# ucl-exoplanets/wayne

Measured on AMD Instinct MI355X. Metric: simulated WFC3-IR exposures/sec (1014x1014, NSAMP=16, spatial scan), higher is better.
Workload: dtype k_ramp<float, true, 1, false, true>: exact integer sums (int64 accumulators + int32 sky counts) then an all-f32 per-read chain; f32 thrower (int32 LDS tiles -> int64 fixed-point accumulators, 2^-28 e-); f32 reads; 1 GPU; cfg4: G141 spatial scan 5 px/s, SUBARRAY=1024 (frame 1014x1014), SPARS10 NSAMP=16, K=128 sub-samples, W=4494 bins, 9.92e+08 electrons/exposure, all detector effects on (flat, sky, cosmic rays, gain, dark, non-linearity, clip, read noise), thrower=split (wide component per electron, narrow component multinomial), f32 reads (the default of ExposureGenerator, Observation, VisitRunner and the CLI), on; exposures_per_rank=2241

## Files before the change

### wayne_amd/_lib.py

```python
import ctypes as C
import os
import threading
import weakref

import numpy as np

from . import build as _build

OK, E_INVALID, E_NEGATIVE, E_OVERFLOW, E_NOMEM, E_HIP, E_NODEVICE, E_STATE = 0, -1, -2, -3, -4, -5, -6, -7
RNG_REPLAY, RNG_PHILOX, RNG_SPLIT = 0, 1, 2
F_ADD_FLAT = 1 << 0
F_ADD_GAIN_VARIATIONS = 1 << 1
F_ADD_NON_LINEAR = 1 << 2
F_CLIP_DET_LIMITS = 1 << 3
F_ADD_READ_NOISE = 1 << 4
F_ADD_STELLAR_NOISE = 1 << 5
F_ADD_DARK = 1 << 6
F_ADD_INITIAL_BIAS = 1 << 7
F_OUT_F64 = 1 << 16
F_OUT_U16 = 1 << 18
OUT_FLAGS = {np.dtype(np.float32): 0, np.dtype(np.float64): F_OUT_F64, np.dtype(np.uint16): F_OUT_U16}
F_EXACT_SAMPLERS = 1 << 17
PROF_KERNELS = 8
ABI_VERSION = 7
# ... 33 lines not shown


class ExposureDesc(C.Structure):
    _fields_ = [("seed", C.c_uint32), ("exposure_index", C.c_uint32), ("rng_mode", C.c_int),
                ("threads_compat", C.c_int), ("flags", C.c_uint32), ("sub_scale", C.c_int),
                ("n_wl", C.c_int), ("wl_um", _dp), ("flux", _dp), ("depth", _dp),
                ("n_samples", C.c_int), ("x_ref", _dp), ("y_ref", _dp), ("dur_ms", _dp),
                ("replay_seed", _ip), ("sample_read", _ip),
                ("n_reads", C.c_int), ("read_dt_s", _dp),
                ("sky_ct_s", C.c_double), ("cosmic_rate", C.c_double), ("scale_factor", C.c_double),
                ("noise_mean", C.c_double), ("noise_std", C.c_double),
                ("thrower_margin", C.c_int), ("thrower_splits", C.c_int),
                ("lc_z", _dp), ("lc_hidden", _dp), ("lc_rp", _dp), ("lc_ld", C.c_double * 4)]


class SourceDesc(C.Structure):
    _fields_ = [("tag", C.c_uint32), ("n_wl", C.c_int), ("wl_um", _dp), ("flux", _dp),
                ("dx", C.c_double), ("dy", C.c_double)]


class TrapDesc(C.Structure):
    _fields_ = [("n_traps", C.c_double * 2), ("efficiency", C.c_double * 2), ("lifetime_s", C.c_double * 2),
                ("n_rate", C.c_int), ("rate_lo", C.c_double), ("rate_hi", C.c_double), ("start", _dp * 2)]


class ExtractDesc(C.Structure):
    _fields_ = [("steps", C.c_uint32), ("row_lo", C.c_int * EXTRACT_PRODUCTS), ("row_hi", C.c_int * EXTRACT_PRODUCTS),
                ("bg_col_lo", C.c_int), ("bg_col_hi", C.c_int)]


class Profile(C.Structure):
    _fields_ = [("name", C.c_char_p * PROF_KERNELS), ("launches", C.c_uint64 * PROF_KERNELS),
                ("ms", C.c_double * PROF_KERNELS), ("electrons", C.c_uint64)]


_vp = C.c_void_p
SYMBOLS = {
    "wayne_abi_version": (C.c_int, []),
    "wayne_strerror": (C.c_char_p, [C.c_int]),
    "wayne_build_flags": (C.c_char_p, []),
    "wayne_device_count": (C.c_int, []),
    "wayne_ctx_create": (_vp, [C.c_int, C.POINTER(C.c_int)]),
    "wayne_ctx_destroy": (None, [_vp]),
    "wayne_last_error": (C.c_char_p, [_vp]),
    "wayne_ctx_synchronize": (C.c_int, [_vp]),
    "wayne_ctx_stream": (_vp, [_vp]),
    "wayne_ctx_set_knob": (C.c_int, [_vp, C.c_char_p, C.c_longlong]),
    "wayne_ctx_get_knob": (C.c_int, [_vp, C.c_char_p, C.POINTER(C.c_longlong)]),
    "wayne_psf_apply": (C.c_int, [_vp, _vp, C.c_int, _vp, _vp, _vp, _vp, _vp, C.c_int, C.c_int,
                                  C.c_uint32, C.c_int, C.c_int, C.c_uint32, C.c_uint32, _vp]),
    "wayne_psf_apply_ex": (C.c_int, [_vp, _vp, C.c_int, _vp, _vp, _vp, _vp, _vp, C.c_int, C.c_int,
                                     C.c_uint32, C.c_int, C.c_int, C.c_uint32, C.c_uint32, C.c_uint32, _vp]),
    "wayne_ctx_set_grism": (C.c_int, [_vp, C.POINTER(GrismDesc)]),
    "wayne_ctx_set_calibration": (C.c_int, [_vp, C.POINTER(Calibration)]),
    "wayne_ctx_slots": (C.c_int, [_vp]),
    "wayne_exposure_upload": (C.c_int, [_vp, C.c_int, C.POINTER(ExposureDesc)]),
    "wayne_exposure_run": (C.c_int, [_vp, C.c_int]),
    "wayne_exposure_run_checked": (C.c_int, [_vp, C.c_int]),
    "wayne_exposure_status": (C.c_int, [_vp, C.c_int, C.POINTER(C.c_int)]),
    "wayne_ctx_reruns": (C.c_ulonglong, [_vp]),
    "wayne_exposure_download": (C.c_int, [_vp, C.c_int, _vp]),
    "wayne_exposure_fetch_async": (C.c_int, [_vp, C.c_int]),
    "wayne_exposure_wait": (C.c_int, [_vp, C.c_int, C.POINTER(C.c_void_p)]),
    "wayne_exposure_device_reads": (_vp, [_vp, C.c_int]),
    "wayne_exposure_synthesize": (C.c_int, [_vp, C.POINTER(ExposureDesc), _vp]),
    "wayne_exposure_debug_fetch": (C.c_int, [_vp, C.c_int, _vp, _vp, _vp, _vp]),
    "wayne_exposure_debug_depth": (C.c_int, [_vp, C.c_int, _vp]),
    "wayne_exposure_debug_boxes": (C.c_int, [_vp, C.c_int, _vp, _vp, C.POINTER(C.c_int)]),
    "wayne_exposure_run_front": (C.c_int, [_vp, C.c_int]),
    "wayne_exposure_run_back": (C.c_int, [_vp, C.c_int]),
    "wayne_exposure_ramp_variant": (C.c_int, [_vp, C.c_int, C.c_char_p, C.c_int]),
    "wayne_exposure_set_sources": (C.c_int, [_vp, C.c_int, C.POINTER(SourceDesc), C.c_int]),
    "wayne_source_seed": (C.c_uint32, [C.c_uint32, C.c_uint32]),
    "wayne_exposure_set_traps": (C.c_int, [_vp, C.c_int, C.POINTER(TrapDesc)]),
    "wayne_exposure_debug_fetch_source": (C.c_int, [_vp, C.c_int, C.c_int, _vp, _vp, _vp]),
    "wayne_exposure_set_extraction": (C.c_int, [_vp, C.c_int, C.POINTER(ExtractDesc)]),
    "wayne_exposure_fetch_spectra_async": (C.c_int, [_vp, C.c_int]),
    "wayne_exposure_wait_spectra": (C.c_int, [_vp, C.c_int, C.POINTER(_dp), C.POINTER(_dp)]),
    "wayne_exposure_download_spectra": (C.c_int, [_vp, C.c_int, _vp, _vp]),
    "wayne_extract_profile": (C.c_int, [_vp, C.POINTER(C.c_uint64), C.POINTER(C.c_double)]),
    "wayne_profile_enable": (C.c_int, [_vp, C.c_int]),
    "wayne_profile_select": (C.c_int, [_vp, C.c_uint]),
    "wayne_profile_reset": (C.c_int, [_vp]),
    "wayne_profile_get": (C.c_int, [_vp, C.POINTER(Profile)]),
    "wayne_philox4x32": (None, [_vp, _vp, _vp]),
    "wayne_host_sample_draws": (None, [C.c_uint32, C.c_uint32, C.c_int, _vp, _vp, _vp]),
}

_lib = None


def load():
    global _lib, _lib_path
    if _lib is None:
        path = _build.LIB
        override = os.environ.get("WAYNE_HIP_LIB")
        if override:
            path = override
        elif _build.stale():
            if os.path.exists(_build.HIPCC):
                _build.build(verbose=False)
            elif not os.path.exists(path):
                raise ImportError("libwayne_hip.so is not built and hipcc is unavailable (%s)" % _build.HIPCC)
        L = C.CDLL(path)
        for name, (res, args) in SYMBOLS.items():
            f = getattr(L, name)
            f.restype = res
            f.argtypes = args
        if L.wayne_abi_version() != ABI_VERSION:
            raise ImportError("libwayne_hip.so ABI version mismatch")
        flags = L.wayne_build_flags().decode().split()
        if flags and os.environ.get("WAYNE_ALLOW_FLAGGED_LIB", "") != "1":
            raise ImportError("%s was built with %s: not the product's library (tests and measurement scripts that mean "
                              "to load it set WAYNE_ALLOW_FLAGGED_LIB=1)" % (path, " ".join(flags)))
        _lib = L
        _lib_path = path
    return _lib


_lib_path = None


def library_info():
    L = load()
    return _lib_path or _build.LIB, L.wayne_build_flags().decode().strip()


def ptr(a, ctype=None):
    if a is None:
        return None
    assert a.flags["C_CONTIGUOUS"]
    if ctype is None:
        return a.ctypes.data_as(C.c_void_p)
    return a.ctypes.data_as(C.POINTER(ctype))


def out_dtype_of(flags):
    return np.dtype(np.float64 if flags & F_OUT_F64 else np.uint16 if flags & F_OUT_U16 else np.float32)


def f64(a):
    return np.ascontiguousarray(a, dtype=np.float64)


def f32(a):
    return np.ascontiguousarray(a, dtype=np.float32)


def i32(a):
    return np.ascontiguousarray(a, dtype=np.int32)


KNOBS = ("tile_ints", "batch", "thin", "no_acc_box", "lane_reach", "throw_wgs", "keep_narrow", "no_fuse", "fork_narrow",
         "streams", "upload_timing", "ramp_reads")
_live_contexts = weakref.WeakSet()
_knob_defaults = {}


def set_knob_all(name, value):
    if name not in KNOBS:
        raise KeyError("no knob named %r" % (name,))
    if value is None:
        _knob_defaults.pop(name, None)
    else:
        _knob_defaults[name] = int(value)
    for c in list(_live_contexts):
        if getattr(c, "_h", None):
            c.set_knob(name, value)


def reset_knobs_all():
    for name in list(_knob_defaults):
        set_knob_all(name, None)


class Context(object):

    def __init__(self, device=0):
        self._L = load()
        st = C.c_int(0)
        self._h = self._L.wayne_ctx_create(int(device), C.byref(st))
        if not self._h:
            msg = self._L.wayne_strerror(st.value).decode()
            cls = WayneNoDeviceError if st.value == E_NODEVICE else WayneError
            raise cls(st.value, "wayne_ctx_create(device=%d): %s -- the HIP path is the only path, "
                                "there is no CPU fallback" % (device, msg))
        self.device = device
        self._slot_meta = {}
        self._slot_src = {}
        _live_contexts.add(self)
        for name, value in _knob_defaults.items():
            self.set_knob(name, value)

    def close(self):
        if getattr(self, "_h", None):
            self._L.wayne_ctx_destroy(self._h)
            self._h = None

    def __del__(self):
        try:
            self.close()
        except Exception:
            pass

    def __enter__(self):
        return self

    def __exit__(self, *a):
        self.close()

    def check(self, status):
        if status != OK:
            raise WayneError(status, self._L.wayne_last_error(self._h).decode())

    def synchronize(self):
        self.check(self._L.wayne_ctx_synchronize(self._h))

    def set_knob(self, name, value):
        self.check(self._L.wayne_ctx_set_knob(self._h, name.encode(), -1 if value is None else int(value)))

    def get_knob(self, name):
        v = C.c_longlong(0)
        self.check(self._L.wayne_ctx_get_knob(self._h, name.encode(), C.byref(v)))
        return None if v.value < 0 else int(v.value)

    @property
    def stream(self):
        return self._L.wayne_ctx_stream(self._h)

    def psf_apply(self, counts, x, y, ratio, sl, sh, nr, nc, seed, threads=1, rng_mode=RNG_REPLAY,
                  exposure=0, subsample=0, exact_samplers=False):
        counts = i32(counts)
        x, y, ratio, sl, sh = f64(x), f64(y), f64(ratio), f64(sl), f64(sh)
        n = counts.size
        if not all(a.size == n for a in (x, y, ratio, sl, sh)):
            raise ValueError("apply_psf: arrays differ in length")
        out = np.empty(max(int(nr) * int(nc), 0), dtype=np.int32)
        self.check(self._L.wayne_psf_apply_ex(self._h, ptr(counts), n, ptr(x), ptr(y), ptr(ratio), ptr(sl),
                                              ptr(sh), int(nr), int(nc), int(seed) & 0xFFFFFFFF, int(threads),
                                              int(rng_mode), int(exposure), int(subsample),
                                              F_EXACT_SAMPLERS if exact_samplers else 0, ptr(out)))
        return out

    def set_grism(self, trace_coeff, wl_solution, psf_ratio_poly, psf_sigmal_poly, psf_sigmah_poly,
                  sens_wl_um, sens_val, flat_wmin, flat_wmax):
        g = GrismDesc()
        g.trace_coeff[:] = list(map(float, trace_coeff))
        g.wl_solution[:] = list(map(float, wl_solution))
        g.psf_ratio_poly[:] = list(map(float, psf_ratio_poly))
        g.psf_sigmal_poly[:] = list(map(float, psf_sigmal_poly))
        g.psf_sigmah_poly[:] = list(map(float, psf_sigmah_poly))
        wl, val = f64(sens_wl_um), f64(sens_val)
        if wl.size != val.size:
            raise ValueError("sensitivity table: wl and val differ in length")
        g.n_sens = wl.size
        g.sens_wl_um = ptr(wl, C.c_double)
        g.sens_val = ptr(val, C.c_double)
        g.flat_wmin, g.flat_wmax = float(flat_wmin), float(flat_wmax)
        self.check(self._L.wayne_ctx_set_grism(self._h, C.byref(g)))

    def set_calibration(self, subarray, n_reads, flat=None, pfl=None, sky=None, lin=None, dark_sci=None,
                        dark_err=None, zero_read=None):
        N = 1014 if subarray == 1024 else subarray
        S = N + 10
        k = Calibration()
        k.subarray, k.n_reads = int(subarray), int(n_reads)
        keep = []

        def plane(a, shape, name, dt=np.float32):
            a = np.ascontiguousarray(a, dtype=dt)
            if a.shape != shape:
                raise ValueError("%s: expected shape %s, got %s" % (name, shape, a.shape))
            keep.append(a)
            return a

        if flat is not None:
            for i in range(4):
                k.flat[i] = ptr(plane(flat[i], (N, N), "flat[%d]" % i), C.c_float)
        if pfl is not None:
            k.pfl = ptr(plane(pfl, (N, N), "pfl"), C.c_float)
        if sky is not None:
            k.sky = ptr(plane(sky, (N, N), "sky"), C.c_float)
        if lin is not None:
            for i in range(4):
                k.lin[i] = ptr(plane(lin[i], (S, S), "lin[%d]" % i), C.c_float)
        if dark_sci is not None and dark_err is not None:
            k.dark_sci = ptr(plane(dark_sci, (n_reads, S, S), "dark_sci"), C.c_float)
            k.dark_err = ptr(plane(dark_err, (n_reads, S, S), "dark_err"), C.c_float)
        if zero_read is not None:
            k.zero_read = ptr(plane(zero_read, (S, S), "zero_read", np.float64), C.c_double)
        self.check(self._L.wayne_ctx_set_calibration(self._h, C.byref(k)))
        self.N, self.S, self.R = N, S, int(n_reads)

    def make_desc(self, *a, **k):
        return make_desc(*a, **k)

    def upload(self, slot, desc):
        self.check(self._L.wayne_exposure_upload(self._h, int(slot), C.byref(desc)))
        self._slot_meta[slot] = (desc.n_samples, desc.n_wl, desc.n_reads, out_dtype_of(desc.flags))
        self._slot_src[slot] = ()
        sources = getattr(desc, "_sources", None)
        if sources:
            self.set_sources(slot, sources)
        traps = getattr(desc, "_traps", None)
        if traps is not None:
            self.set_traps(slot, traps)
        extraction = getattr(desc, "_extraction", None)
# ... 266 lines not shown
```

### wayne_amd/csrc/k_narrow.h

```cpp
#pragma once
#include "common.h"
#include "k_throw.h"

namespace wayne {

constexpr int kNarrowCells = 2 * kNarrowR + 1;
constexpr int kPoolRows = 2 * kNarrowR + 2;
constexpr int kNarrowTile = 1536;

constexpr float kTailCut = 6.5f;
template <class M>
__device__ __forceinline__ float upper_tail(float t) {
  if (__all(t > kTailCut)) return 0.f;
  const float z = t * 0.70710678118654752f;
  const float u = M::div_(1.f, 1.f + 0.5f * z);
  float p = 0.17087277f;
  p = fmaf(p, u, -0.82215223f);
  p = fmaf(p, u, 1.48851587f);
  p = fmaf(p, u, -1.13520398f);
  p = fmaf(p, u, 0.27886807f);
  p = fmaf(p, u, -0.18628806f);
  p = fmaf(p, u, 0.09678418f);
  p = fmaf(p, u, 0.37409196f);
  p = fmaf(p, u, 1.00002368f);
  p = fmaf(p, u, -1.26551223f);
  p = fmaf(-z, z, p);
  return (t > kTailCut) ? 0.f : (0.5f * u) * M::exp_(p);
}

template <int FLUSH, bool FAST>
__global__ __launch_bounds__(kNarrowThreads) void k_narrow(ThrowArgs a) {
  typedef typename std::conditional<FAST, FastMath, ExactMath<float> >::type M;
  __shared__ int tile[kNarrowTile];
  __shared__ float s_q[kPoolRows][kNarrowThreads];
  __shared__ int s_pool[kNarrowThreads];
  __shared__ float s_cond[kNarrowThreads];
  __shared__ int s_box[4];
  __shared__ float s_fc[10];
  if (threadIdx.x < 10) s_fc[threadIdx.x] = (float)kStirlingSmall[threadIdx.x];
  const int k = blockIdx.x;
  const int tid = threadIdx.x;
  const uint32_t order_word = reinterpret_cast<const uint32_t*>(a.chunk_order)[blockIdx.y >> 2];
  const int w = (int)((order_word >> (8 * (blockIdx.y & 3))) & 0xFFu) * kNarrowThreads + tid;
  const SubInfo si = a.sub[k];
  int n0 = 0;
  double xd = 0., yd = 0., sgd = 1.;
  if (w < a.W) {
    const size_t kw = (size_t)k * a.W + w;
    n0 = a.nsplit[kw];
    xd = a.xpos[kw];
    yd = a.ypos[kw];
    sgd = a.sigl[w];
  }
  if (!__syncthreads_or(n0 > 0)) return;
  const bool split = n0 > 0;
  BinLocal bl{};
  if (split) bl = bin_local(xd, yd);
  const bool act = split && bl.sane;
  const float sg = split ? (float)sgd : 1.f;
  const int ic0 = bl.ox, jc0 = bl.oy;
  s_pool[tid] = 0;
  if (tid == 0) { s_box[0] = 0x7FFFFFFF; s_box[1] = -0x7FFFFFFF; s_box[2] = 0x7FFFFFFF; s_box[3] = -0x7FFFFFFF; }
  __syncthreads();
  {
    const int x_lo = wave_mini(act ? ic0 - kNarrowR : 0x7FFFFFFF), x_hi = wave_maxi(act ? ic0 + kNarrowR + 1 : -0x7FFFFFFF);
    const int y_lo = wave_mini(act ? jc0 - kNarrowR : 0x7FFFFFFF), y_hi = wave_maxi(act ? jc0 + kNarrowR + 1 : -0x7FFFFFFF);
    if ((tid & 63) == 0) {
      atomicMin(&s_box[0], x_lo); atomicMax(&s_box[1], x_hi);
      atomicMin(&s_box[2], y_lo); atomicMax(&s_box[3], y_hi);
    }
  }
  __syncthreads();
  int tx0 = max(s_box[0], 1), tx1 = min(s_box[1], a.N), ty0 = max(s_box[2], 1), ty1 = min(s_box[3], a.N);
  int tw = max(tx1 - tx0, 0), th = max(ty1 - ty0, 0);
  if ((long long)tw * th > kNarrowTile) { th = min(th, kNarrowTile / max(tw, 1)); if (th < 1) { th = 0; tw = 0; } }
  const int tarea = tw * th;
  for (int i = tid; i < tarea; i += kNarrowThreads) tile[i] = 0;

  auto deposit = [&](int ci, int rj, int m) {
    const int lx = ci - tx0, ly = rj - ty0;
    if ((unsigned)lx < (unsigned)tw && (unsigned)ly < (unsigned)th)
      atomicAdd(&tile[ly * tw + lx], m);
    else if (ci > 0 && ci < a.N && rj > 0 && rj < a.N)
      deposit_global<FLUSH>(a, si, ci, rj, m);
  };

  const bool any_multi = __any(act);
  const float inv_s = 1.f / sg;
  const int grp = tid & ~15, gl = tid & 15;
  bool pool = false;
  int X0 = 0, J0 = 0, res = 0;
  float Z = 1.f, Rb = 0.f, yl = 0.f;
  if (any_multi) {
    const int cnt = row16_sum(split ? 1 : 0), cnt_sane = row16_sum(act ? 1 : 0), tot = row16_sum(split ? n0 : 0);
    const int icmin = row16_mini(act ? ic0 : 0x7FFFFFFF), icmax = row16_maxi(act ? ic0 : -0x7FFFFFFF);
    const int jcmin = row16_mini(act ? jc0 : 0x7FFFFFFF);
    X0 = icmin - kNarrowR;
    J0 = jcmin - kNarrowR;
    yl = act ? (float)(yd - (double)J0) : 0.f;
    const float ymin = row16_min(act ? yl : 3e38f), ymax = row16_max(act ? yl : -3e38f);
    const float smin = row16_min(split ? sg : 3e38f), smax = row16_max(split ? sg : 0.f);
    pool = cnt >= 2 && cnt_sane == cnt && icmax - icmin <= 2 && (ymax - ymin) <= 0.25f * smin && smax <= 1.1f * smin &&
           tot <= 16777216;

    float qh[kPoolRows];
#pragma unroll
    for (int t = 0; t < kPoolRows; ++t) qh[t] = 3e38f;
    if (act && pool) {
      float Ep = -yl, Ap = upper_tail<M>(fabsf(Ep) * inv_s), S = 0.f;
#pragma unroll
      for (int t = 0; t < kPoolRows; ++t) {
        const float E = (float)(t + 1) - yl, A = upper_tail<M>(fabsf(E) * inv_s);
        const float m = (Ep >= 0.f) ? Ap - A : ((E <= 0.f) ? A - Ap : 1.f - Ap - A);
        qh[t] = fmaxf(m, 0.f);
        S += qh[t];
        Ep = E; Ap = A;
      }
#pragma unroll
      for (int t = 0; t < kPoolRows; ++t) qh[t] = M::div_(qh[t], S);
    } else if (act) {
      const float f = bl.fy;
      float up = upper_tail<M>((1.f - f) * inv_s), lo = upper_tail<M>(f * inv_s);
      s_q[0][tid] = 1.f - up - lo;
      for (int c = 1; c < kNarrowCells; ++c) {
        const int d = (c + 1) >> 1;
        const float rem = up + lo;
        float Q;
        if (c & 1) { const float nx = upper_tail<M>(((float)(d + 1) - f) * inv_s); Q = up - nx; up = nx; }
        else       { const float nx = upper_tail<M>(((float)d + f) * inv_s);       Q = lo - nx; lo = nx; }
        s_q[c][tid] = fminf(fmaxf(M::div_(Q, rem), 0.f), 1.f);
      }
    }
    if (__any(pool)) {
      float qb[kPoolRows];
#pragma unroll
      for (int t = 0; t < kPoolRows; ++t) qb[t] = row16_min(qh[t]);
      float PL[kNarrowR + 1], SU[kPoolRows + 1];
      PL[0] = qb[0];
#pragma unroll
      for (int t = 1; t <= kNarrowR; ++t) PL[t] = PL[t - 1] + qb[t];
      SU[kPoolRows] = 0.f;
#pragma unroll
      for (int t = kPoolRows - 1; t > kNarrowR; --t) SU[t] = SU[t + 1] + qb[t];
      Z = fminf(PL[kNarrowR] + SU[kNarrowR + 1], 1.f);
      if (act && pool) {
#pragma unroll
        for (int t = 0; t < kPoolRows; ++t) {
          Rb += qh[t] - qb[t];
          s_q[t][tid] = Rb;
        }
      }
      if (pool && gl == 0) {
        s_cond[grp] = fminf(fmaxf(M::div_(qb[kNarrowR], PL[kNarrowR] + SU[kNarrowR + 1]), 0.f), 1.f);
#pragma unroll
        for (int i = 1; i < kPoolRows; ++i) {
          const int u = (i + 1) >> 1;
          float rem, q;
          if (i & 1) { q = qb[kNarrowR + u]; rem = SU[kNarrowR + u] + (u <= kNarrowR ? PL[u <= kNarrowR ? kNarrowR - u : 0] : 0.f); }
          else       { q = qb[kNarrowR - u]; rem = SU[kNarrowR + 1 + u] + PL[kNarrowR - u]; }
          s_cond[grp + i] = fminf(fmaxf(M::div_(q, rem), 0.f), 1.f);
        }
      }
    }
  }
  __syncthreads();

  if (any_multi) {
    SeededStream rng(a.seed, STAGE_NARROW, (uint32_t)w, (uint32_t)k + a.subsample0, a.exposure);
    const float fx = bl.fx;
    float up = upper_tail<M>((1.f - fx) * inv_s), lo = upper_tail<M>(fx * inv_s);
    float n_rem = act ? (float)n0 : 0.f;
    for (int c = __any(pool) ? -1 : 0; c < kNarrowCells; ++c) {
      if (!__any(n_rem > 0.f)) break;
      const int d = (c + 1) >> 1;
      const int ci = (c <= 0) ? ic0 : ((c & 1) ? ic0 + d : ic0 - d);
      float P, rem;
      if (c < 0) { P = Z; rem = 1.f; }
      else if (c == 0) { P = 1.f - up - lo; rem = 1.f; }
      else if (c & 1) { const float nx = upper_tail<M>(((float)(d + 1) - fx) * inv_s); P = up - nx; rem = up + lo; up = nx; }
      else            { const float nx = upper_tail<M>(((float)d + fx) * inv_s);       P = lo - nx; rem = up + lo; lo = nx; }
      float n_col = 0.f;
      if (n_rem > 0.f && (c >= 0 || pool)) {
        const float pc = (c < 0) ? P : fminf(fmaxf(M::div_(P, rem), 0.f), 1.f);
#ifdef WAYNE_TIMING_COLPOOL
        if (c >= 0 && (tid >> 6) >= 2) n_col = fminf(floorf(fmaf(n_rem, pc, 0.5f)), n_rem);
        else
#endif
        n_col = binomial<M>(n_rem, pc, rng, s_fc);
        if (c < 0) { res = (int)(n_rem - n_col); n_rem = n_col; n_col = 0.f; }
        else n_rem -= n_col;
      }
      if (pool) {
        if (n_col > 0.f) atomicAdd(&s_pool[grp + (ci - X0)], (int)n_col);
        n_col = 0.f;
      }
      if (!__any(n_col > 0.f)) continue;
      float m_rem = n_col;
      for (int r = 0; r < kNarrowCells; ++r) {
        if (!__any(m_rem > 0.f)) break;
        float m = 0.f;
        if (m_rem > 0.f) {
          m = binomial<M>(m_rem, s_q[r][tid], rng, s_fc);
          m_rem -= m;
        }
        if (m > 0.f) {
          const int e = (r + 1) >> 1;
          deposit(ci, (r == 0) ? jc0 : ((r & 1) ? jc0 + e : jc0 - e), (int)m);
        }
      }
    }
    if (__any(res > 0)) {
      const float cs = (-1.3862943611198906f * sg) * sg;
      for (int e = 0; __any(e < res); ++e) {
        if (e < res) {
          uint32_t wa, wb, va, vb;
          rng.next2(wa, wb);
          rng.next2(va, vb);
          const float Rs = __builtin_amdgcn_sqrtf(cs * __builtin_amdgcn_logf(u01f(wb)));
          const int col = ic0 + min(max(floor_to_int(fmaf(__builtin_amdgcn_cosf(rev12(wa)), Rs, fx)), -kNarrowR), kNarrowR);
          const float u = u01f(va) * Rb;
          int row = 0;
#pragma unroll
          for (int t = 0; t < kPoolRows - 1; ++t) row += (u >= s_q[t][tid]) ? 1 : 0;
          deposit(col, J0 + row, 1);
        }
      }
    }
    if (__any(pool)) {
      __builtin_amdgcn_fence(__ATOMIC_RELEASE, "wavefront");
      __builtin_amdgcn_wave_barrier();
      __builtin_amdgcn_fence(__ATOMIC_ACQUIRE, "wavefront");
      float left = pool ? (float)s_pool[tid] : 0.f;
      if (__any(left > 0.f)) {
        SeededStream rp(a.seed, STAGE_POOL, (uint32_t)w >> 4, (uint32_t)k + a.subsample0, a.exposure, (uint32_t)gl);
        for (int i = 0; i < kPoolRows; ++i) {
          if (!__any(left > 0.f)) break;
          float m = 0.f;
          if (left > 0.f) {
            m = binomial<M>(left, s_cond[grp + i], rp, s_fc);
            left -= m;
          }
          if (m > 0.f) {
            const int u = (i + 1) >> 1;
            deposit(X0 + gl, J0 + ((i & 1) ? kNarrowR + u : kNarrowR - u), (int)m);
          }
        }
      }
    }
  }
  __syncthreads();
  for (int i = tid; i < tarea; i += kNarrowThreads) {
    const int n = tile[i];
    if (n > 0) {
      const int ly = i / tw, lx = i - ly * tw;
      deposit_global<FLUSH>(a, si, tx0 + lx, ty0 + ly, n);
    }
  }
}

constexpr int kLaneMargin = 30;
constexpr int kLaneReachMax = 48;
constexpr int kLaneTile = 9216;


template <int FLUSH, bool THIN, bool BATCH, bool FUSED>
__device__ __forceinline__ void lane_body(const ThrowArgs& a, const PrepArgs& p, const CosmicArgs& ca) {
  __shared__ int tile[kLaneTile];
  __shared__ SubInfo s_sub[FUSED ? kLaneBatchMax : 1];
  __shared__ uint32_t s_hits;
  __shared__ unsigned short s_list[THIN ? kLaneListCap : 1];
  __shared__ int s_cnt[2];
  __shared__ int s_box[4];
  __shared__ int s_reach;
  const int k0 = BATCH ? (int)blockIdx.x * a.kb : (int)blockIdx.x, k1 = BATCH ? min(k0 + a.kb, a.K) : k0 + 1;
  const int tid = threadIdx.x;
  const uint32_t order_word = reinterpret_cast<const uint32_t*>(a.lane_order)[blockIdx.y >> 2];
  const int w = (int)((order_word >> (8 * (blockIdx.y & 3))) & 0xFFu) * kLaneThreads + tid;
  const bool inw = w < a.W;
  int n_one = 0, nw_one = 0;
  BinLocal bl_one{};
  float ch = 0.f, cl = 0.f, sh = 0.f, sl = 0.f;
  if (inw) {
    double sh_d = a.sigh[w], sl_d = a.sigl[w];
    if (!FUSED && !BATCH) {
      const size_t kw0 = (size_t)k0 * a.W + w;
      n_one = a.nlane[kw0];
      const double xd = a.xpos[kw0], yd = a.ypos[kw0];
      nw_one = a.nwide[kw0];
      bl_one = bin_local(xd, yd);
      nw_one = min(max(nw_one, 0), n_one);
    }
    sh = (float)sh_d; sl = (float)sl_d;
    ch = (-1.3862943611198906f * sh) * sh;
    cl = (-1.3862943611198906f * sl) * sl;
  }
  const bool bad_h = !(ch > -3e38f), bad_l = !(cl > -3e38f);
  if (bad_h) ch = 0.f;
  if (bad_l) cl = 0.f;
  double f_wl = 0., f_flux = 0., f_sens = 0., f_dlam = 0., f_ratio = 0., f_sigl = 0.;
  unsigned long long f_electrons = 0ull;
  if (FUSED) {
    if (ca.rate >= 0.) {
      const int n_wg = gridDim.x * gridDim.y;
      for (int r = blockIdx.y * gridDim.x + blockIdx.x; r < ca.R; r += n_wg) { cosmic_hits(ca, r, &s_hits); __syncthreads(); }
    }
    if (inw) { f_wl = p.wl[w]; f_flux = p.flux[w]; f_sens = p.wa.sens[w]; f_dlam = p.wa.dlam[w]; f_ratio = p.wa.ratio[w]; f_sigl = p.wa.sigl[w]; }
    if (tid < k1 - k0) {
      const int k = k0 + tid;
      s_sub[tid] = make_sub_info(p, k, p.x_ref[k], p.y_ref[k], p.tr + kTrStride * (size_t)k, 0u, 1e300, -1e300, 1e300, -1e300);
    }
  }
  int x_lo = 0x7FFFFFFF, x_hi = -0x7FFFFFFF, y_lo = 0x7FFFFFFF, y_hi = -0x7FFFFFFF;
  float reach = 0.f;
  bool any = false;
  for (int k = k0; k < k1; ++k) {
    const size_t kw = (size_t)k * a.W + (inw ? w : 0);
    int n = 0, nw = 0;
    int ic = 0, jc = 0;
    bool sane = false;
    if (FUSED) {
      if (inw) {
        float x = 0.f, y = 0.f;
        bin_position_bound(p, f_wl, p.tr + kTrStride * (size_t)k, p.x_ref[k], p.y_ref[k], &x, &y);
        sane = fabsf(x) < 1e6f && fabsf(y) < 1e6f;
        ic = (int)floorf(x); jc = (int)floorf(y);
        n = 2; nw = 1;
      }
    } else if (!BATCH) {
      n = n_one;
      if (n > 0) { sane = bl_one.sane; ic = bl_one.ox; jc = bl_one.oy; nw = nw_one; }
    } else if (inw) {
      n = a.nlane[kw];
      if (n > 0) {
        const BinLocal b = bin_local(a.xpos[kw], a.ypos[kw]);
        sane = b.sane; ic = b.ox; jc = b.oy;
        nw = min(max(a.nwide[kw], 0), n);
      }
    }
    if (n > 0) {
      any = true;
      const bool sig_ok = (nw > 0 ? (sh >= 0.f && sh < 1e6f) : true) && (n > nw ? (sl >= 0.f && sl < 1e6f) : true);
      const float smax = fmaxf(nw > 0 ? sh : 0.f, n > nw ? sl : 0.f);
      float r = sig_ok ? 6.9f * smax + 1.f : __int_as_float(0x7F800000);
      if (sane) {
        constexpr int spare = FUSED ? 1 : 0;
        x_lo = min(x_lo, ic - spare); x_hi = max(x_hi, ic + spare); y_lo = min(y_lo, jc - spare); y_hi = max(y_hi, jc + spare);
      } else {
        r = __int_as_float(0x7F800000);
      }
      reach = fmaxf(reach, r);
    }
  }
  if (!__syncthreads_or(any)) return;
  if (tid == 0) { s_box[0] = 0x7FFFFFFF; s_box[1] = -0x7FFFFFFF; s_box[2] = 0x7FFFFFFF; s_box[3] = -0x7FFFFFFF; s_reach = 0; s_cnt[0] = 0; s_cnt[1] = 0; }
  __syncthreads();
  {
    x_lo = wave_mini(x_lo); x_hi = wave_maxi(x_hi); y_lo = wave_mini(y_lo); y_hi = wave_maxi(y_hi);
    const int r_hi = wave_maxi(__float_as_int(reach));
    if ((tid & 63) == 0) {
      atomicMin(&s_box[0], x_lo); atomicMax(&s_box[1], x_hi);
      atomicMin(&s_box[2], y_lo); atomicMax(&s_box[3], y_hi);
      atomicMax(&s_reach, r_hi);
    }
  }
  __syncthreads();
  const float reach_wg = __int_as_float(s_reach);
  bool sure = reach_wg <= (float)kLaneReachMax;
  const int margin = sure ? (int)ceilf(reach_wg) : kLaneMargin;
  const int bx0 = s_box[0] - margin, bx1 = s_box[1] + margin + 1, by0 = s_box[2] - margin, by1 = s_box[3] + margin + 1;
  int tx0 = max(bx0, 1), tx1 = min(bx1, a.N), ty0 = max(by0, 1), ty1 = min(by1, a.N);
  int tw = max(tx1 - tx0, 0), th = max(ty1 - ty0, 0);
  sure = sure && s_box[0] <= s_box[1] && tx0 == bx0 && tx1 == bx1 && ty0 == by0 && ty1 == by1 && (long long)tw * th <= kLaneTile;
  while ((long long)tw * th > kLaneTile && th > 1) { ty0 += 1; th = max(th - 2, 1); }
  while ((long long)tw * th > kLaneTile && tw > 1) { tx0 += 1; tw = max(tw - 2, 1); }
  if ((long long)tw * th > kLaneTile) { tw = 0; th = 0; }
  const int tarea = tw * th;
  for (int i = tid; i < tarea; i += kLaneThreads) tile[i] = 0;

  int par = 0;
  auto tile_add = [&](int addr) {
    if (THIN) {
      if (atomicAdd((int*)((char*)tile + addr), 1) == 0) {
        const unsigned long long m = __ballot(1);
        const int before = __builtin_amdgcn_mbcnt_hi((unsigned)(m >> 32), __builtin_amdgcn_mbcnt_lo((unsigned)m, 0u));
        int base = 0;
        if (before == 0) base = atomicAdd(&s_cnt[par], __popcll(m));
        base = __builtin_amdgcn_readfirstlane(base);
        if (base + before < kLaneListCap) s_list[base + before] = (unsigned short)(addr >> 2);
      }
    } else {
      atomicAdd((int*)((char*)tile + addr), 1);
    }
  };

  for (int k = k0; k < k1; ++k) {
  const size_t kw = (size_t)k * a.W + (inw ? w : 0);
  int n = 0, nw = 0;
// ... 163 lines not shown
```

### wayne_amd/csrc/wayne_hip.hip

```cpp
#include "../../include/wayne_hip.h"

#include <hip/hip_runtime.h>
#include <hip/hip_ext.h>

#include <algorithm>
#include <chrono>
#include <cmath>
#include <cstdio>
#include <cstdlib>
#include <cstring>
#include <map>
#include <new>
#include <string>
#include <vector>

#include "kernels.h"
#include "host_plan.h"

using namespace wayne;

struct wayne_ctx;

namespace {

// ... 36 lines not shown
  void view(void* at) {
    if (owns && p) (void)hipFree(p);
    p = at;
    cap = 0;
    owns = false;
  }
  template <class T> T* as() const { return (T*)p; }
};

struct PinnedBuf {
  char* p = nullptr;
  size_t cap = 0;
  PinnedBuf() = default;
  PinnedBuf(const PinnedBuf&) = delete;
  PinnedBuf& operator=(const PinnedBuf&) = delete;
  ~PinnedBuf() { if (p) (void)hipHostFree(p); }
  bool reserve(size_t bytes) {
    if (bytes <= cap) return true;
    if (p) (void)hipHostFree(p);
    p = nullptr;
    cap = 0;
    if (hipHostMalloc((void**)&p, bytes, hipHostMallocDefault) != hipSuccess) { p = nullptr; return false; }
    cap = bytes;
    return true;
  }
};

struct StageArena {
  PinnedBuf host;
  DevBuf dev;
  hipEvent_t ev = nullptr;
  bool pending = false;
  size_t used = 0;
  ~StageArena() { if (ev) (void)hipEventDestroy(ev); }
  int begin(wayne_ctx* c, size_t bytes, const char* nomem_msg, bool with_event = true) {
    if (pending) { HIP_TRY(c, hipEventSynchronize(ev)); pending = false; }
    if (!host.reserve(align64(bytes))) return fail(c, WAYNE_E_NOMEM, nomem_msg);
    if (with_event && !ev) HIP_TRY(c, hipEventCreateWithFlags(&ev, hipEventDisableTiming));
    HIP_TRY(c, dev.reserve(host.cap));
    used = 0;
    return WAYNE_OK;
  }
  char* place(DevBuf& view, size_t bytes) {
    bytes = std::max<size_t>(bytes, 1);
    if (used + bytes > host.cap) return nullptr;
    char* h = host.p + used;
    view.view((char*)dev.p + used);
    used += align64(bytes);
    return h;
  }
  bool put(DevBuf& view, const void* src, size_t bytes) {
    char* h = place(view, bytes);
    if (h && bytes) std::memcpy(h, src, bytes);
    return h != nullptr;
  }
  int commit(wayne_ctx* c, hipStream_t stream) {
    HIP_TRY(c, hipMemcpyAsync(dev.p, host.p, used, hipMemcpyHostToDevice, stream));
    if (ev) { HIP_TRY(c, hipEventRecord(ev, stream)); pending = true; }
    return WAYNE_OK;
  }
  template <class T> const T* host_of(const DevBuf& view) const { return (const T*)(host.p + ((const char*)view.p - (const char*)dev.p)); }
};

struct SourceState {
  bool fused_last = false;
  PrepArgs last_prep{};
  int last_chunks = 0;
  int W = 0;
  uint32_t seed = 0;
  DevBuf wl, flux, xref, yref;
  DevBuf ratio, sigl, sigh, sens, dlam;
  DevBuf counts, nwide, nsplit, nlane, prefix, xpos, ypos, sub, chunk_total, chunk_box, tr;
  int kb = 1;
  bool thin = false;
  double max_narrow = 0.;
  double max_chunk_electrons = 0.;
  double est_thrown = 0.;
  unsigned char chunk_order[kMaxChunks] = {0};
  unsigned char lane_order[kMaxChunks] = {0};
  StageArena src_stage;
};

constexpr int kMaxSources = WAYNE_MAX_SOURCES;

struct Slot : SourceState {
  bool uploaded = false;
  bool front_done = false;
  bool acc_dirty = false;
  bool acc_init = false;
  bool force_throw = false;
  bool ran = false;
  wayne_exposure_desc d{};
  int K = 0, R = 0;
  bool has_depth = false, has_replay_seed = false, has_lc = false, has_lc_hidden = false;
  DevBuf depth, dur, rseed, sread, read_dt, lc_z, lc_hidden, lc_rp;
  int n_extra = 0;
  SourceState extra[kMaxSources];
  uint32_t extra_tag[kMaxSources] = {0};
  SourceState& source(int i) { return i == 0 ? *this : extra[i - 1]; }
  DevBuf acc, out, misc;
  DevBuf seg;
  bool use_box = false;
  int acc_box[16][4] = {{0}};
  PinnedBuf pinned;
  struct Misc { unsigned long long electrons; int status; int pad; };
  Misc* pinned_misc = nullptr;
  StageArena sky_stage;
  DevBuf sky_tab;
  std::vector<uint32_t> sky_tab_keys;
  bool sky_alias_on = false, sky_pieces = false;
  uint32_t sky_mask = 0;
  int sky_L = 1;
  float sky_level[16] = {0};
  unsigned char sky_tab0[16] = {0};
  std::vector<double> read_dt_host;
  double lc_p_lo = 0., lc_p_hi = 0.;
  bool traps_on = false;
  double trap_n[2] = {1., 1.}, trap_eta[2] = {0., 0.}, trap_tau[2] = {1., 1.}, trap_lo = 0., trap_hi = 0.;
  int trap_G = 0;
  StageArena trap_stage;
  DevBuf trap_d, trap_f;
  bool extract_on = false;
  wayne_extract_desc ex{};
  int ex_chunks = 0;
  DevBuf ex_part, ex_out;
  PinnedBuf ex_pinned;
  Misc* ex_pinned_misc = nullptr;
  StageArena stage;
};

struct ProfRec {
  int kernel;
  hipEvent_t a, b;
};

constexpr int kSlots = 256;

}

constexpr int kStreams = 2;

struct Knobs {
  long long tile_ints = -1;
  long long batch = -1;
  long long thin = -1;
  long long no_acc_box = -1;
  long long lane_reach = -1;
  long long throw_wgs = -1;
  long long keep_narrow = -1;
  long long no_fuse = -1;
  long long fork_narrow = -1;
  long long streams = -1;
  long long upload_timing = -1;
  long long ramp_reads = -1;
};
struct KnobName { const char* name; const char* env; long long Knobs::*field; };
const KnobName kKnobNames[] = {
    {"tile_ints", "WAYNE_TILE_INTS", &Knobs::tile_ints},       {"batch", "WAYNE_BATCH", &Knobs::batch},
    {"thin", "WAYNE_THIN", &Knobs::thin},                      {"no_acc_box", "WAYNE_NO_ACC_BOX", &Knobs::no_acc_box},
    {"lane_reach", "WAYNE_LANE_REACH", &Knobs::lane_reach},    {"throw_wgs", "WAYNE_THROW_WGS", &Knobs::throw_wgs},
    {"keep_narrow", "WAYNE_KEEP_NARROW", &Knobs::keep_narrow}, {"no_fuse", "WAYNE_NO_FUSE", &Knobs::no_fuse},
    {"fork_narrow", "WAYNE_FORK_NARROW", &Knobs::fork_narrow}, {"streams", "WAYNE_STREAMS", &Knobs::streams},
    {"upload_timing", "WAYNE_UPLOAD_TIMING", &Knobs::upload_timing}, {"ramp_reads", "WAYNE_RAMP_READS", &Knobs::ramp_reads},
};
constexpr size_t kMiscBytes = 64;

constexpr size_t kCounterBytes = (size_t)kCounterStripes * kCounterStride * sizeof(unsigned long long);

struct CtxStreams {
  hipStream_t stream = nullptr;
  hipStream_t streams[kStreams] = {nullptr, nullptr};
  hipStream_t side[kStreams] = {nullptr, nullptr};
  hipEvent_t ev_fork[kStreams] = {nullptr, nullptr}, ev_join[kStreams] = {nullptr, nullptr};
  bool fork_narrow = true;
  hipEvent_t ev_kdone[kStreams] = {nullptr, nullptr};
  bool kdone_valid[kStreams] = {false, false};
  ~CtxStreams() {
    for (int i = 0; i < kStreams; ++i) {
      if (streams[i]) (void)hipStreamDestroy(streams[i]);
      if (side[i]) (void)hipStreamDestroy(side[i]);
      if (ev_fork[i]) (void)hipEventDestroy(ev_fork[i]);
      if (ev_join[i]) (void)hipEventDestroy(ev_join[i]);
      if (ev_kdone[i]) (void)hipEventDestroy(ev_kdone[i]);
    }
  }
};

struct wayne_ctx : CtxStreams {
  int device = 0;
  int n_streams = kStreams;
  Knobs knobs;
  DevBuf status_all;
  PinnedBuf status_host;
  std::string err;
  bool have_grism = false;
  GrismDev g{};
  DevBuf sens_wl, sens_val;
  plan::SpectrumEstimate est;
  plan::SpectrumEstimate src_est[kMaxSources];
  bool have_cal = false;
  int subarray = 0, N = 0, S = 0, cal_R = 0;
  DevBuf flat[4], pfl, sky, lin[4], dark_sci, dark_err, zero_read;
  bool has_flat = false, has_pfl = false, has_sky = false, has_lin = false, has_dark = false,
       has_zero = false;
  float sky_max = 0.f, sky_min = 0.f;
  std::vector<float> sky_sorted;
  double up_us[6] = {0, 0, 0, 0, 0, 0};
  long up_calls = 0;
  Slot slots[kSlots];
  DevBuf pa_prefix, pa_nwide, pa_nsplit, pa_nlane, pa_x, pa_y, pa_sl, pa_sh, pa_sub, pa_frame;
  StageArena pa_stage;
  bool prof_on = false;
  unsigned prof_mask = ~0u;
  std::vector<ProfRec> prof;
  std::vector<hipEvent_t> ev_pool;
  uint64_t prof_launches[kProfKernels] = {0};
  double prof_ms[kProfKernels] = {0};
  uint64_t electrons = 0;
  uint64_t reruns = 0;
  DevBuf counters;
};

namespace {

void plan_lanes(const wayne_ctx* c, SourceState& ss, int K, int W) {
  int kb = 1;
  plan::lane_batches(K, W, ss.max_chunk_electrons, &kb, &ss.thin);
  {
    if (c->knobs.batch >= 0) kb = (int)std::min<long long>(std::max<long long>(c->knobs.batch, 1), kLaneBatchMax);
    if (c->knobs.thin >= 0) ss.thin = c->knobs.thin != 0;
  }
  ss.kb = kb;
}

int reserve_source(wayne_ctx* c, SourceState& ss, int K, int W) {
  const size_t KW = (size_t)K * W, n_chunks = (size_t)(W + kPrepThreads - 1) / kPrepThreads;
  for (DevBuf* b : {&ss.ratio, &ss.sigl, &ss.sigh, &ss.sens, &ss.dlam}) HIP_TRY(c, b->reserve((size_t)W * sizeof(double)));
  for (DevBuf* b : {&ss.counts, &ss.nwide, &ss.nsplit, &ss.nlane}) HIP_TRY(c, b->reserve(KW * sizeof(int32_t)));
  HIP_TRY(c, ss.prefix.reserve((size_t)K * (W + 1) * sizeof(uint32_t)));
  HIP_TRY(c, ss.xpos.reserve(KW * sizeof(double)));
  HIP_TRY(c, ss.ypos.reserve(KW * sizeof(double)));
  HIP_TRY(c, ss.sub.reserve((size_t)K * sizeof(SubInfo)));
  HIP_TRY(c, ss.tr.reserve((size_t)K * kTrStride * sizeof(double)));
  HIP_TRY(c, ss.chunk_total.reserve(K * n_chunks * sizeof(uint32_t)));
  HIP_TRY(c, ss.chunk_box.reserve(K * n_chunks * 4 * sizeof(double)));
  return WAYNE_OK;
}

void adopt_plan(const wayne_ctx* c, SourceState& ss, int K, int W, const plan::ThrowPlan& tp) {
  ss.est_thrown = tp.est_thrown; ss.max_chunk_electrons = tp.max_chunk_electrons; ss.max_narrow = tp.max_narrow;
  std::memcpy(ss.chunk_order, tp.chunk_order, sizeof ss.chunk_order);
  std::memcpy(ss.lane_order, tp.lane_order, sizeof ss.lane_order);
  plan_lanes(c, ss, K, W);
}

int fail(wayne_ctx* c, int code, const std::string& msg) {
  if (c) c->err = msg;
  return code;
}

hipEvent_t get_event(wayne_ctx* c) {
  if (!c->ev_pool.empty()) {
    hipEvent_t e = c->ev_pool.back();
    c->ev_pool.pop_back();
    return e;
  }
  hipEvent_t e = nullptr;
  if (hipEventCreate(&e) != hipSuccess) return nullptr;
  return e;
}

struct ProfScope {
  wayne_ctx* c;
  ProfRec rec{};
  bool on;
  bool ext = false;
  ProfScope(wayne_ctx* c_, int kernel, bool ext_launch = false) : c(c_), on(c_->prof_on && ((c_->prof_mask >> kernel) & 1u)) {
    if (!on) return;
    rec.kernel = kernel;
    rec.a = get_event(c);
    rec.b = get_event(c);
    if (!rec.a || !rec.b) { on = false; return; }
    ext = ext_launch;
    if (!ext) (void)hipEventRecord(rec.a, c->stream);
  }
  ~ProfScope() {
    if (!on) return;
    if (!ext) (void)hipEventRecord(rec.b, c->stream);
    c->prof.push_back(rec);
  }
};

int sync_all(wayne_ctx* c) {
  for (int i = 0; i < kStreams; ++i) {
    HIP_TRY(c, hipStreamSynchronize(c->streams[i]));
    if (c->side[i]) HIP_TRY(c, hipStreamSynchronize(c->side[i]));
  }
  return WAYNE_OK;
}

void use_slot_stream(wayne_ctx* c, int slot) { c->stream = c->streams[slot % c->n_streams]; }

int collect_profile(wayne_ctx* c) {
  int rc = sync_all(c);
  if (rc) return rc;
  for (ProfRec& r : c->prof) {
    float ms = 0.f;
    if (hipEventElapsedTime(&ms, r.a, r.b) == hipSuccess) {
      c->prof_ms[r.kernel] += ms;
      c->prof_launches[r.kernel] += 1;
    }
    c->ev_pool.push_back(r.a);
    c->ev_pool.push_back(r.b);
  }
  c->prof.clear();
  return WAYNE_OK;
}

template <class T>
int upload(wayne_ctx* c, DevBuf& b, const T* src, size_t n) {
  HIP_TRY(c, b.reserve(std::max<size_t>(n, 1) * sizeof(T)));
  if (n) HIP_TRY(c, hipMemcpyAsync(b.p, src, n * sizeof(T), hipMemcpyHostToDevice, c->stream));
  return WAYNE_OK;
}

using plan::build_sky_alias;

template <class T>
int upload_staged(wayne_ctx* c, Slot& s, DevBuf& b, const T* src, size_t n) {
  if (!s.stage.put(b, src, n * sizeof(T))) return fail(c, WAYNE_E_NOMEM, "upload: staging arena too small");
  return WAYNE_OK;
}

int prepare_sky_tables(wayne_ctx* c, Slot& s) {
  const wayne_exposure_desc& d = s.d;
  plan::SkyPlan sp;
  plan::plan_sky(d.sky_ct_s, s.R, s.read_dt_host.data(), c->has_sky, c->sky_min, c->sky_max, c->sky_sorted, &sp);
  s.sky_pieces = sp.pieces; s.sky_alias_on = false; s.sky_mask = 0; s.sky_L = 1;
  for (int l = 0; l < 16; ++l) { s.sky_level[l] = sp.level[l]; s.sky_tab0[l] = sp.tab0[l]; }
  if (!sp.alias_on) { s.sky_pieces = false; return WAYNE_OK; }
  if (sp.keys != s.sky_tab_keys || !s.sky_tab.p) {
    const size_t bytes = (size_t)kMaxReads * kSkyAlias * sizeof(uint32_t);
    int rc = s.sky_stage.begin(c, bytes, "upload: pinned allocation for the sky tables failed");
    if (rc) return rc;
    uint32_t* tab = (uint32_t*)s.sky_stage.place(s.sky_tab, bytes);
    std::memset(tab, 0, bytes);
    for (size_t t = 0; t < sp.keys.size() && t < (size_t)kMaxReads; ++t) {
      float lam;
      std::memcpy(&lam, &sp.keys[t], 4);
      build_sky_alias((double)lam, tab + t * kSkyAlias);
    }
    if ((rc = s.sky_stage.commit(c, c->stream))) return rc;
    s.sky_tab_keys = sp.keys;
  }
  s.sky_alias_on = true;
  s.sky_mask = sp.mask;
  s.sky_L = sp.L;
  return WAYNE_OK;
}

int side_of(int subarray) { return subarray == 1024 ? 1014 : subarray; }

std::vector<float> embed(const float* src, int N, int S, float fill) {
  std::vector<float> v((size_t)S * S, fill);
  for (int y = 0; y < N; ++y)
    std::memcpy(&v[(size_t)(y + kBorder) * S + kBorder], src + (size_t)y * N, (size_t)N * sizeof(float));
  return v;
}

int thrower_lds_ints(const wayne_ctx* c, int splits, int margin) {
  if (c->knobs.tile_ints >= 0) return (int)std::min<long long>(std::max<long long>(c->knobs.tile_ints, 256), 40000);
  const long long w = 260 / std::max(splits, 1) + 2 * margin + 4, h = 2 * margin + 12;
  return (int)std::min<long long>(std::max<long long>(w * h, 1024), 12288);
}

template <int RNG, int FLUSH>
int launch_throw(wayne_ctx* c, const ThrowArgs& a, int lds_ints) {
  const int groups = (a.K + 7) / 8;
  const dim3 grid((unsigned)(a.K < 8 ? a.K * a.splits : groups * 8 * a.splits));
  const size_t lds = (size_t)lds_ints * sizeof(int);
  HIP_TRY(c, hipFuncSetAttribute((const void*)k_throw<RNG, FLUSH>,
                                 hipFuncAttributeMaxDynamicSharedMemorySize, (int)lds));
  hipLaunchKernelGGL((k_throw<RNG, FLUSH>), grid, dim3(kThrowThreads), lds, c->stream, a);
  HIP_TRY(c, hipGetLastError());
  return WAYNE_OK;
}

template <int FLUSH>
int launch_narrow(wayne_ctx* c, const ThrowArgs& a, bool exact) {
  const dim3 grid((unsigned)a.K, (unsigned)((a.W + kNarrowThreads - 1) / kNarrowThreads));
  if (exact) hipLaunchKernelGGL((k_narrow<FLUSH, false>), grid, dim3(kNarrowThreads), 0, c->stream, a);
  else hipLaunchKernelGGL((k_narrow<FLUSH, true>), grid, dim3(kNarrowThreads), 0, c->stream, a);
  HIP_TRY(c, hipGetLastError());
  return WAYNE_OK;
}

int out_kind(uint32_t flags) { return (flags & WAYNE_F_OUT_F64) ? 1 : (flags & WAYNE_F_OUT_U16) ? 2 : 0; }
size_t out_elem_size(uint32_t flags) {
  const int k = out_kind(flags);
  return k == 1 ? sizeof(double) : k == 2 ? sizeof(uint16_t) : sizeof(float);
}

template <class OutT, bool FAST, int SKY, bool NOISE>
void (*ramp_kernel())(RampArgs) {
  if constexpr (FAST && SKY != 0 && !NOISE) return k_ramp<OutT, FAST, SKY, NOISE>;
  else return k_ramp_wide<OutT, FAST, SKY, NOISE>;
}
template <class OutT, bool FAST, int SKY>
void (*ramp_noise(bool noise))(RampArgs) { return noise ? ramp_kernel<OutT, FAST, SKY, true>() : ramp_kernel<OutT, FAST, SKY, false>(); }
template <class OutT, bool FAST>
void (*ramp_sky(int sky, bool noise))(RampArgs) {
  return sky == 1 ? ramp_noise<OutT, FAST, 1>(noise) : sky == 2 ? ramp_noise<OutT, FAST, 2>(noise) : ramp_noise<OutT, FAST, 0>(noise);
}
void (*pick_ramp(int out, bool exact, int sky, bool noise))(RampArgs) {
  return out == 1 ? (exact ? ramp_sky<double, false>(sky, noise) : ramp_sky<double, true>(sky, noise))
       : out == 2 ? (exact ? ramp_sky<uint16_t, false>(sky, noise) : ramp_sky<uint16_t, true>(sky, noise))
                  : (exact ? ramp_sky<float, false>(sky, noise) : ramp_sky<float, true>(sky, noise));
}

template <int FLUSH>
int launch_lane(wayne_ctx* c, const ThrowArgs& a, bool thin, const PrepArgs* fused_prep = nullptr, const CosmicArgs* fused_cosmic = nullptr) {
  const dim3 grid((unsigned)((a.K + a.kb - 1) / a.kb), (unsigned)((a.W + kLaneThreads - 1) / kLaneThreads));
  if (fused_prep) {
    hipLaunchKernelGGL((k_lane_fused<FLUSH>), grid, dim3(kLaneThreads), 0, c->stream, a, *fused_prep, *fused_cosmic);
  } else if (a.kb > 1) {
    if (thin) hipLaunchKernelGGL((k_lane<FLUSH, true, true>), grid, dim3(kLaneThreads), 0, c->stream, a);
    else hipLaunchKernelGGL((k_lane<FLUSH, false, true>), grid, dim3(kLaneThreads), 0, c->stream, a);
  } else {
    if (thin) hipLaunchKernelGGL((k_lane<FLUSH, true, false>), grid, dim3(kLaneThreads), 0, c->stream, a);
    else hipLaunchKernelGGL((k_lane<FLUSH, false, false>), grid, dim3(kLaneThreads), 0, c->stream, a);
  }
  HIP_TRY(c, hipGetLastError());
  return WAYNE_OK;
}


typedef void (*RampTrapKernel)(RampArgs, TrapArgs);
template <class OutT, bool FAST, int SKY>
RampTrapKernel trap_noise(bool noise) { return noise ? k_ramp_trap<OutT, FAST, SKY, true, false> : k_ramp_trap<OutT, FAST, SKY, false, false>; }
template <class OutT, bool FAST>
RampTrapKernel trap_sky(int sky, bool noise) {
  return sky == 1 ? trap_noise<OutT, FAST, 1>(noise) : sky == 2 ? trap_noise<OutT, FAST, 2>(noise) : trap_noise<OutT, FAST, 0>(noise);
}
RampTrapKernel pick_ramp_trap(int out, bool exact, int sky, bool noise, bool allon) {
  if (allon) return out == 2 ? k_ramp_trap<uint16_t, true, 1, false, true> : k_ramp_trap<float, true, 1, false, true>;
  return out == 1 ? (exact ? trap_sky<double, false>(sky, noise) : trap_sky<double, true>(sky, noise))
       : out == 2 ? (exact ? trap_sky<uint16_t, false>(sky, noise) : trap_sky<uint16_t, true>(sky, noise))
                  : (exact ? trap_sky<float, false>(sky, noise) : trap_sky<float, true>(sky, noise));
}

void (*select_ramp(const wayne_ctx* c, const Slot& s, std::string* name, RampTrapKernel* trap = nullptr))(RampArgs) {
  const wayne_exposure_desc& d = s.d;
  const int out = out_kind(d.flags);
  const bool f64 = out == 1, exact = (d.flags & WAYNE_F_EXACT_SAMPLERS) != 0;
  const char* out_name = out == 1 ? "double" : out == 2 ? "unsigned short" : "float";
  const int sky_mode = !s.sky_alias_on ? 0 : (s.sky_pieces ? 2 : 1);
  const bool noise = d.noise_mean != 0. && d.noise_std != 0.;
  void (*kern)(RampArgs) = pick_ramp(out, exact, sky_mode, noise);
  const uint32_t all_on = WAYNE_F_ADD_DARK | WAYNE_F_ADD_NON_LINEAR | WAYNE_F_CLIP_DET_LIMITS | WAYNE_F_ADD_READ_NOISE;
  const bool allon = !f64 && !exact && sky_mode == 1 && !noise && (d.flags & all_on) == all_on && c->has_dark && c->has_lin;
  if (allon) kern = out == 2 ? k_ramp<uint16_t, true, 1, false, true> : k_ramp<float, true, 1, false, true>;
  if (trap) *trap = s.traps_on ? pick_ramp_trap(out, exact, sky_mode, noise, allon) : nullptr;
  if (name) {
    const bool pinned = !exact && sky_mode != 0 && !noise;
    char buf[96];
    if (s.traps_on)
      std::snprintf(buf, sizeof buf, "k_ramp_trap<%s, %s, %d, %s, %s>", out_name, exact ? "false" : "true",
                    sky_mode, noise ? "true" : "false", allon ? "true" : "false");
    else
      std::snprintf(buf, sizeof buf, "%s<%s, %s, %d, %s%s>", pinned ? "k_ramp" : "k_ramp_wide", out_name,
                    exact ? "false" : "true", sky_mode, noise ? "true" : "false", pinned ? (allon ? ", true" : ", false") : "");
    *name = buf;
  }
  return kern;
}

int launch_extract(wayne_ctx* c, Slot& s) {
  const int S = c->S, R = s.R;
  ExtractArgs a{};
  a.R = R; a.S = S;
  a.steps = s.ex.steps;
  a.bg_lo = s.ex.bg_col_lo; a.bg_hi = s.ex.bg_col_hi;
  a.n_chunks = s.ex_chunks;
  double sum_dt = 0.;
  for (int j = 0; j < R; ++j) { a.scale[j] = s.read_dt_host[j]; sum_dt += s.read_dt_host[j]; }
  a.scale[R] = sum_dt;
  for (int j = 0; j <= R; ++j) { a.row_lo[j] = s.ex.row_lo[j]; a.row_hi[j] = s.ex.row_hi[j]; }
  a.reads = s.out.p;
  a.pfl = c->has_pfl ? c->pfl.as<float>() : nullptr;
  a.sky = c->has_sky ? c->sky.as<float>() : nullptr;
  for (int i = 0; i < 4; ++i) a.lin[i] = c->has_lin ? c->lin[i].as<float>() : nullptr;
  a.dark = c->has_dark ? c->dark_sci.as<float>() : nullptr;
  a.part = s.ex_part.as<double>();
  a.spectra = s.ex_out.as<double>();
  a.sky_out = s.ex_out.as<double>() + (size_t)(R + 1) * S;
  const int products = (a.steps & X_LAST_READ) ? R + 1 : R;
  for (int p = 0; p <= kExtractProducts; ++p) a.first_chunk[p] = 0;
  for (int p = 0; p < products; ++p)
    a.first_chunk[p + 1] = a.first_chunk[p] + (a.row_hi[p] - a.row_lo[p] + kExtractRows - 1) / kExtractRows;
  for (int p = products; p < kExtractProducts; ++p) a.first_chunk[p + 1] = a.first_chunk[p];
  const dim3 grid((unsigned)((S + 63) / 64), (unsigned)a.first_chunk[products]);
  ProfScope ps(c, PK_EXTRACT);
  const int out = out_kind(s.d.flags);
  if (out == 1) hipLaunchKernelGGL((k_extract_rows<double>), grid, dim3(kExtractThreads), 0, c->stream, a);
  else if (out == 2) hipLaunchKernelGGL((k_extract_rows<uint16_t>), grid, dim3(kExtractThreads), 0, c->stream, a);
  else hipLaunchKernelGGL((k_extract_rows<float>), grid, dim3(kExtractThreads), 0, c->stream, a);
  HIP_TRY(c, hipGetLastError());
  hipLaunchKernelGGL(k_extract_finish, dim3((unsigned)(R + 1)), dim3(kExtractThreads), 0, c->stream, a);
  HIP_TRY(c, hipGetLastError());
  return WAYNE_OK;
}

}

namespace {
bool box_empty(const int* b) { return b[0] >= b[1] || b[2] >= b[3]; }
}

extern "C" {

int wayne_abi_version(void) { return WAYNE_ABI_VERSION; }

const char* wayne_strerror(int s) {
  switch (s) {
    case WAYNE_OK: return "ok";
    case WAYNE_E_INVALID: return "invalid argument";
    case WAYNE_E_NEGATIVE: return "negative electron count";
    case WAYNE_E_OVERFLOW: return "electron count overflows the reference's int arithmetic";
    case WAYNE_E_NOMEM: return "out of memory";
    case WAYNE_E_HIP: return "HIP runtime error";
    case WAYNE_E_NODEVICE: return "no gfx950 device";
    case WAYNE_E_STATE: return "grism / calibration / upload missing";
    default: return "unknown status";
  }
}

int wayne_device_count(void) {
  int n = 0;
  if (hipGetDeviceCount(&n) != hipSuccess) return 0;
  return n;
}

wayne_ctx* wayne_ctx_create(int device, int* status) {
  auto set = [&](int s) { if (status) *status = s; };
  int n = 0;
// ... 1254 lines not shown
```

Baseline: 3082 exposures/s.

## Compact live pool lanes by size class before narrow binomial sampling

Adds a compacted path for the narrow kernel's multinomial pool stage. Threads with a nonzero pool are bucketed by log2 of their count with an LDS histogram and prefix scan, then packed densely into the first wavefronts, sorted largest class first, before running the per-row binomial loop. The aim is to cut wavefront divergence and idle lanes in that loop. It costs extra block-wide barriers, LDS atomics and a scan, and it reuses s_q as scratch. The path is on by default because the knob defaults to -1, which counts as nonzero.

Measured after the change: 3143 exposures/s (median of 6 runs). +2.0%, better.

```diff
diff --git a/wayne_amd/_lib.py b/wayne_amd/_lib.py
--- a/wayne_amd/_lib.py
+++ b/wayne_amd/_lib.py
@@ -209,7 +209,7 @@
 
 
 KNOBS = ("tile_ints", "batch", "thin", "no_acc_box", "lane_reach", "throw_wgs", "keep_narrow", "no_fuse", "fork_narrow",
-         "streams", "upload_timing", "ramp_reads")
+         "streams", "upload_timing", "ramp_reads", "narrow_compact")
 _live_contexts = weakref.WeakSet()
 _knob_defaults = {}
 
diff --git a/wayne_amd/csrc/k_narrow.h b/wayne_amd/csrc/k_narrow.h
--- a/wayne_amd/csrc/k_narrow.h
+++ b/wayne_amd/csrc/k_narrow.h
@@ -28,7 +28,7 @@
   return (t > kTailCut) ? 0.f : (0.5f * u) * M::exp_(p);
 }
 
-template <int FLUSH, bool FAST>
+template <int FLUSH, bool FAST, bool COMPACT>
 __global__ __launch_bounds__(kNarrowThreads) void k_narrow(ThrowArgs a) {
   typedef typename std::conditional<FAST, FastMath, ExactMath<float> >::type M;
   __shared__ int tile[kNarrowTile];
@@ -37,7 +37,9 @@
   __shared__ float s_cond[kNarrowThreads];
   __shared__ int s_box[4];
   __shared__ float s_fc[10];
+  __shared__ int s_gx[COMPACT ? kNarrowThreads / 16 : 1], s_gj[COMPACT ? kNarrowThreads / 16 : 1], s_hist[COMPACT ? 32 : 1];
   if (threadIdx.x < 10) s_fc[threadIdx.x] = (float)kStirlingSmall[threadIdx.x];
+  if (COMPACT && threadIdx.x < 32) s_hist[threadIdx.x] = 0;
   const int k = blockIdx.x;
   const int tid = threadIdx.x;
   const uint32_t order_word = reinterpret_cast<const uint32_t*>(a.chunk_order)[blockIdx.y >> 2];
@@ -226,7 +228,7 @@
         }
       }
     }
-    if (__any(pool)) {
+    if (!COMPACT && __any(pool)) {
       __builtin_amdgcn_fence(__ATOMIC_RELEASE, "wavefront");
       __builtin_amdgcn_wave_barrier();
       __builtin_amdgcn_fence(__ATOMIC_ACQUIRE, "wavefront");
@@ -243,6 +245,50 @@
           if (m > 0.f) {
             const int u = (i + 1) >> 1;
             deposit(X0 + gl, J0 + ((i & 1) ? kNarrowR + u : kNarrowR - u), (int)m);
+          }
+        }
+      }
+    }
+  }
+  if (COMPACT) {
+    __builtin_amdgcn_fence(__ATOMIC_RELEASE, "wavefront");
+    __builtin_amdgcn_wave_barrier();
+    __builtin_amdgcn_fence(__ATOMIC_ACQUIRE, "wavefront");
+    const int mine = pool ? s_pool[tid] : 0;
+    if (gl == 0) { s_gx[tid >> 4] = X0; s_gj[tid >> 4] = J0; }
+    if (__syncthreads_or(mine > 0)) {
+      int* const list = reinterpret_cast<int*>(&s_q[0][0]);
+      const int cls = (mine > 0) ? 31 - __clz(mine) : 0;
+      int rank = 0;
+      if (mine > 0) rank = atomicAdd(&s_hist[cls], 1);
+      __syncthreads();
+      const int lane = tid & 63;
+      const int h = (lane < 32) ? s_hist[31 - lane] : 0;
+      int incl = h;
+#pragma unroll
+      for (int off = 1; off < 32; off <<= 1) {
+        const int v = __shfl_up(incl, off);
+        if (lane >= off) incl += v;
+      }
+      const int first = __shfl(incl - h, 31 - cls), n_live = __shfl(incl, 31);
+      if (mine > 0) list[first + rank] = tid;
+      __syncthreads();
+      if ((tid & ~63) < n_live) {
+        const int slot = (tid < n_live) ? list[tid] : 0;
+        float left = (tid < n_live) ? (float)s_pool[slot] : 0.f;
+        const int cgrp = slot & ~15, cl = slot & 15;
+        const int cX = s_gx[slot >> 4] + cl, cJ0 = s_gj[slot >> 4];
+        SeededStream rp(a.seed, STAGE_POOL, (uint32_t)(w - tid + slot) >> 4, (uint32_t)k + a.subsample0, a.exposure, (uint32_t)cl);
+        for (int i = 0; i < kPoolRows; ++i) {
+          if (!__any(left > 0.f)) break;
+          float m = 0.f;
+          if (left > 0.f) {
+            m = binomial<M>(left, s_cond[cgrp + i], rp, s_fc);
+            left -= m;
+          }
+          if (m > 0.f) {
+            const int u = (i + 1) >> 1;
+            deposit(cX, cJ0 + ((i & 1) ? kNarrowR + u : kNarrowR - u), (int)m);
           }
         }
       }
diff --git a/wayne_amd/csrc/wayne_hip.hip b/wayne_amd/csrc/wayne_hip.hip
--- a/wayne_amd/csrc/wayne_hip.hip
+++ b/wayne_amd/csrc/wayne_hip.hip
@@ -212,6 +212,7 @@
   long long fork_narrow = -1;
   long long streams = -1;
   long long upload_timing = -1;
+  long long narrow_compact = -1;
   long long ramp_reads = -1;
 };
 struct KnobName { const char* name; const char* env; long long Knobs::*field; };
@@ -222,6 +223,7 @@
     {"keep_narrow", "WAYNE_KEEP_NARROW", &Knobs::keep_narrow}, {"no_fuse", "WAYNE_NO_FUSE", &Knobs::no_fuse},
     {"fork_narrow", "WAYNE_FORK_NARROW", &Knobs::fork_narrow}, {"streams", "WAYNE_STREAMS", &Knobs::streams},
     {"upload_timing", "WAYNE_UPLOAD_TIMING", &Knobs::upload_timing}, {"ramp_reads", "WAYNE_RAMP_READS", &Knobs::ramp_reads},
+    {"narrow_compact", "WAYNE_NARROW_COMPACT", &Knobs::narrow_compact},
 };
 constexpr size_t kMiscBytes = 64;
 
@@ -449,8 +451,10 @@
 template <int FLUSH>
 int launch_narrow(wayne_ctx* c, const ThrowArgs& a, bool exact) {
   const dim3 grid((unsigned)a.K, (unsigned)((a.W + kNarrowThreads - 1) / kNarrowThreads));
-  if (exact) hipLaunchKernelGGL((k_narrow<FLUSH, false>), grid, dim3(kNarrowThreads), 0, c->stream, a);
-  else hipLaunchKernelGGL((k_narrow<FLUSH, true>), grid, dim3(kNarrowThreads), 0, c->stream, a);
+  const bool compact = c->knobs.narrow_compact != 0;
+  void (*kern)(ThrowArgs) = exact ? (compact ? k_narrow<FLUSH, false, true> : k_narrow<FLUSH, false, false>)
+                                  : (compact ? k_narrow<FLUSH, true, true> : k_narrow<FLUSH, true, false>);
+  hipLaunchKernelGGL(kern, grid, dim3(kNarrowThreads), 0, c->stream, a);
   HIP_TRY(c, hipGetLastError());
   return WAYNE_OK;
 }
```
